# schumacherlab/ONT-TCRconsensus

Hardware: AMD Instinct MI355X
Metric: UMIs clustered/sec + banded-NW GCUPS (whole node, 1/2/4/8 MI355X) (higher is better)
Workload: dtype int16/int32

## Files before the change

ont-tcrconsensus_amd/csrc/cluster_ctx.h:

```cpp
#pragma once
#include <hip/hip_runtime.h>

#include <atomic>
#include <cstdlib>
#include <cstring>
#include <memory>
#include <thread>
#include <utility>
#include <vector>

#include "ctx.h"
#include "plan.h"
#include "resolve.h"

struct umiclust_ctx;

namespace uc {

constexpr int32_t kDelta = 8192;
constexpr int32_t kDepth = 2;
constexpr int32_t kBlockMin = 2048;
constexpr int32_t kDirectRecQ = 4096;
constexpr int32_t kSpecThr = 30;
constexpr int32_t kLazyPermille = 5;
constexpr int32_t kRbDirect = 4096;

struct DebugSums {
  struct {
    double wait = 0, hq_copy = 0, rec_copy = 0, classify = 0, inorder = 0, enqueue = 0, total = 0, appends = 0,
           round_b = 0, resolve_block = 0;
  } t;
  struct {
    double dev_s = 0, trips = 0, launches = 0, pairs = 0;
  } rb;
  int64_t mispredicted = 0, saved = 0, blocked = 0;
  int64_t q_no_record = 0, q_earlier_only = 0, q_in_block = 0, q_host_ns = 0;
  int64_t s_inline = 0, s_many_relevant = 0, s_record_read = 0, s_peers_scanned = 0;
};

struct Tile {
  DevBuf<uint32_t> hist;
  DevBuf<uint32_t> off;
  DevBuf<uint32_t> cursor;
  DevBuf<uint32_t> partial;
  uint64_t post_base = 0;
  size_t post_cap = 0;
  int32_t n = 0;
  int32_t base = 0;
  int32_t seg = 0;
  int32_t len = 0;
  int32_t built_n = -1;
  bool prebuilt = false;
};

struct Pass {
  int32_t q0 = 0, nq = 0, w0 = 0;
  bool live = false;
  bool rec_direct = false;
  PinBuf<TileView> h_tiles;
  DevBuf<TileView> d_tiles;
  DevBuf<uint32_t> d_top_seqno;
  DevBuf<uint8_t> d_top_count, d_ntop;
  DevBuf<uint32_t> d_pcand, d_units;
  DevBuf<uint8_t> d_pncand, d_ppeer_count, d_pnpeer;
  DevBuf<uint32_t> d_ppost;
  DevBuf<uint16_t> d_ppeer_id;
  DevBuf<uint16_t> d_peer_id;
  DevBuf<uint8_t> d_peer_count, d_npeer;
  bool ctr_zeroed = false;
  DevBuf<uint32_t> d_counters;
// ... 80 lines not shown
  std::vector<int32_t> bin_s;
  int32_t cur_bin = -1;

  DevBuf<char> d_ascii;
  DevBuf<int64_t> d_offs;
  DevBuf<int32_t> d_perm;
  DevBuf<uint32_t> d_codes;
  DevBuf<uint8_t> d_lens;
  DevBuf<uint16_t> d_kmers;
  DevBuf<uint8_t> d_nk;
  DevBuf<char> d_masked;
  DevBuf<int32_t> d_iota;
  size_t iota_n = 0;
  bool staged = false;
  std::vector<uint32_t> rec_len;
  PinBuf<int32_t> h_perm;
  DevBuf<uint32_t> d_amb;
  PinBuf<uint32_t> h_amb;
  int64_t n_changed = 0;
  DevBuf<uint8_t> d_mchg;
  PinBuf<uint16_t> h_xm;
  DevBuf<uint16_t> d_xm;
  std::vector<int32_t> hqbin;
  DevBuf<int32_t> d_qbin, d_bin_seq0, d_bin_ord0;
  PinBuf<int32_t> h_bin_ord0;
  bool pack_on = false;
  DevBuf<uint8_t> d_acc;
  DevBuf<uint16_t> d_rank;
  std::vector<uint8_t> h_acc;
  std::vector<uint16_t> h_rank;
  uc::Index ix{this};
  uc::Pass pass[uc::kPeerTiles];
  uc::Tile blk_tile[uc::kPeerTiles + 1], solo_tile;
  uc::Tile round_tile[2];
  uc::Event a_ev[4][2];
  hipStream_t ix_st = nullptr;
  uc::Event ix_done;
  hipEvent_t last_r_ev = nullptr;
  std::unique_ptr<uc::WorkPool> pool;
  std::thread in_release;
  void join_release() {
    if (in_release.joinable()) in_release.join();
  }
  int32_t pass_B = 0;
  uc::Stream st_b, st_copy;
  PinBuf<uint32_t> h_bpq, h_bpt, h_bres;
  uc::Stream st_al;
  int32_t last_a_slot = -1;
  uc::Event evb[2];
  DevBuf<uint32_t> d_bpq, d_bpt, d_bres;

  std::vector<int32_t> cno;
  std::vector<uint8_t> strand;
  std::vector<int32_t> target;
  std::vector<int32_t> ocl;
  int32_t nclusters = 0;
  uc::ClusterNumbers num;
  std::vector<char> cons;
  std::vector<int64_t> cons_off;
  struct BinOut {
    bool done = false;
    int32_t K = 0;
    std::vector<char> cons;
    std::vector<int64_t> cons_off;
  };
  std::vector<BinOut> bout;
  bool rec_direct = false;
// ... 39 lines not shown

namespace uc {

extern std::atomic<int> g_live_ctx;

int affinity_cpus();
int pool_threads(const umiclust_ctx* c);
hipError_t main_stream_priority(umiclust_ctx* c, int level);
void ensure_traceback_buffers(umiclust_ctx* c, int32_t n);
void launch_tracebacks(umiclust_ctx* c, const DevSeqs& ds, const Scoring& sc, const TracePlan& tp, int32_t maxl,
                       hipStream_t stq);
void ensure_consensus_inputs(umiclust_ctx* c, int32_t n, int32_t K);
constexpr const char* kConsOverMsg = "consensus: %d clusters exceed the MSA column budget";
int32_t run_consensus(umiclust_ctx* c, const DevSeqs& ds, int32_t n, int32_t K, hipEvent_t ev);
void cluster_pinned(umiclust_ctx* c, int32_t bin, bool multi_bin = false, int32_t npk = 1);

struct ClusterRun {
  umiclust_ctx* const c;
  const int32_t bin, npk;
  const bool multi_bin;
  const double t0 = now_s();
  const int32_t s0, s1, n;
  std::vector<uint8_t> state_buf;
  StateView state;
  BlockPlan plan;
  std::vector<int32_t> pending;
  std::vector<int32_t> new_cents;
  bool lazy = false;
  double t_pf = 0, t_al = 0, t_host = 0, t_cons = 0;
  int32_t tw_n = 0;
  int32_t tw_maxl = kMaxLen;
  DevSeqs ds{};
  const int32_t T4;
  const int D;

  ClusterRun(umiclust_ctx* ctx, int32_t bin_, int32_t npk_, bool multi)
      : c(ctx), bin(bin_), npk(npk_), multi_bin(multi), s0(ctx->bin_s[bin_]), s1(ctx->bin_s[bin_ + npk_]), n(s1 - s0),
        T4(ctx->o4_T), D(T4 ? 2 : kDepth) {}

  void reset_bin();
  void plan_blocks();
  void alloc_traceback();
  int32_t rstart(int32_t q) const;
  void sync_index(int32_t X);
  void round_window(int32_t q, const Tile** prevs, int& nprev, int slot);
  void keep_new_cents();
  void count_lazy(int32_t k, int32_t ahead);
  void run_alone(int32_t q0, int32_t nq);
  Tile& tile_of(int32_t k) { return c->blk_tile[k % (D + 1)]; }
  void enqueue(int32_t k, int nprev);
  void prebuild_peer(int32_t k);
  void run_whole();
  Tile& stile(int32_t j) { return c->blk_tile[j % (kPeerTiles + 1)]; }
  void build_peer(int32_t j, bool side);
  void second_half(int32_t j, int32_t first, bool after_count, PfCapture* cap = nullptr);
  void count_half(int32_t j, int32_t first, int flag);
  void prime(int32_t r);
  void run_split();
  void run_pipeline();
  void drain();
  void tw_launch(int32_t lo, int32_t hi, hipStream_t stq);
  void trace_members();
  void number();
  void consensus();
  void store_outputs();
  void report_pf_prof();
  void report_debug() const;
  void report();
};

inline size_t tile_cap(int64_t nseq) {
  const int64_t raw = nseq * kMaxKmers;
  return (size_t)((raw + 7 * std::min<int64_t>(kBins, raw) + 64) & ~int64_t(7));
}
void build_tile(umiclust_ctx* c, Tile& t, const int32_t* map, int32_t first, int32_t n, int32_t xoff, int32_t vbase,
                int32_t seg_mod, hipStream_t st = nullptr);
inline TileView view_of(const Tile& t) {
  TileView v;
  v.off = t.off.p;
  v.post_base = t.post_base;
  v.n = t.n;
  v.base = t.base;
  v.seg = t.seg;
  v.len = t.len;
// ... 47 lines not shown
```

ont-tcrconsensus_amd/csrc/driver.cpp:

```cpp
#include <algorithm>
#include <cstdio>
#include <sched.h>

#include "cluster_ctx.h"

using namespace uc;

std::atomic<int> uc::g_live_ctx{0};

int uc::affinity_cpus() {
  cpu_set_t set;
  if (sched_getaffinity(0, sizeof set, &set) != 0) return io::host_cpus();
  return std::max(1, std::min(CPU_COUNT(&set), io::host_cpus()));
}

int uc::pool_threads(const umiclust_ctx* c) {
  const int want = c->tun.resolve_threads > 0 ? c->tun.resolve_threads : (g_live_ctx.load() > 1 ? 4 : 8);
  return std::max(1, std::min(want, affinity_cpus()));
}

namespace {

struct L3Pin {
  cpu_set_t saved;
// ... 101 lines not shown
    c->hip(hipMemcpyAsync(c->h_craw.p, c->t_cons.p, (size_t)K * kConsCap, hipMemcpyDeviceToHost, c->st), "d2h");
  }
  c->hip(hipMemcpyAsync(c->h_over.p, c->t_over.p, 4, hipMemcpyDeviceToHost, c->st), "d2h");
  c->hip(hipStreamSynchronize(c->st), "sync");
  return *c->h_over.p;
}


void ClusterRun::reset_bin() {
  c->pack_on = npk > 1;
  c->cur_bin = bin;
  std::fill(c->cno.begin() + s0, c->cno.begin() + s1, -1);
  std::fill(c->strand.begin() + s0, c->strand.begin() + s1, 0);
  std::fill(c->target.begin() + s0, c->target.begin() + s1, -1);
  c->nclusters = 0;
  c->ix.reset(n);
  c->stats = umiclust_stats{};
  c->stats.n_input = c->bin_in[bin + npk] - c->bin_in[bin];
  if (c->pack_on) {
    for (int32_t b = bin; b < bin + npk; b++) c->h_bin_ord0.p[b] = INT32_MAX;
    c->hip(hipMemcpyAsync(c->d_bin_ord0.p + bin, c->h_bin_ord0.p + bin, (size_t)npk * 4, hipMemcpyHostToDevice, c->st),
           "h2d bin ord0");
  }
  c->stats.n_kept = n;
  state_buf.assign((size_t)n, ST_UNDET);
  state = StateView{state_buf.data(), s0};
  if (c->tun.walk_dump) c->wd.assign((size_t)n * 4, -1);
}

void ClusterRun::plan_blocks() {
  int32_t B = std::max(1, std::min<int32_t>(c->tun.block_size, kMaxBlock));
  if (c->tun.block_div > 0) B = std::min<int32_t>(B, std::max<int32_t>(kBlockMin, ((s1 - s0) / c->tun.block_div + 255) & ~255));
  c->pass_B = B;
  for (Pass& P : c->pass) ensure_pass_buffers(c, P, B);
  plan.hlen = c->hlen.data();
  plan.s0 = s0;
  plan.s1 = s1;
  plan.B = B;
  plan.mix = c->tun.mix_len > 0 || (c->tun.mix_len < 0 && (B < kMaxBlock || c->pack_on));
  plan.o4_T = T4;
  plan.hqbin = c->pack_on ? c->hqbin.data() : nullptr;
  plan.bin_s = c->bin_s.data();
  plan.regrow = c->tun.regrow;
  plan.start(c->b_hint);
}

void ClusterRun::alloc_traceback() {
  c->t_opsidx.assign(n, -1);
  ensure_traceback_buffers(c, n);
  ds = dev_seqs(c);
  tw_maxl = traceback_maxl(c->hlen.data(), s0, s1);
}

int32_t ClusterRun::rstart(int32_t q) const { return round_start(c, s0, q); }
void ClusterRun::sync_index(int32_t X) {
  size_t m = 0;
  while (m < pending.size() && pending[m] < X) m++;
  if (!m) return;
  std::vector<int32_t> a(pending.begin(), pending.begin() + (ptrdiff_t)m);
  c->ix.append(a);
  pending.erase(pending.begin(), pending.begin() + (ptrdiff_t)m);
}
void ClusterRun::round_window(int32_t q, const Tile** prevs, int& nprev, int slot) {
  const int32_t first = nprev ? prevs[0]->base : q;
  const int32_t W = rstart(first);
  if (W < first) {
    Tile& rt = c->round_tile[slot & 1];
    build_tile(c, rt, c->d_iota.p, W, first - W, 0, (kPeerTiles - 1) * kPeerRegion, 1 << 30);
    rt.base = W;
    rt.seg = kPeerTiles - 1;
    rt.len = 0;
    rt.prebuilt = false;
    for (int i = nprev; i > 0; i--) prevs[i] = prevs[i - 1];
    prevs[0] = &rt;
    nprev++;
  }
  sync_index(W);
}

void ClusterRun::keep_new_cents() {
  if (T4) pending.insert(pending.end(), new_cents.begin(), new_cents.end());
  else c->ix.append(new_cents);
  c->stats.n_blocks++;
}
void ClusterRun::count_lazy(int32_t k, int32_t ahead) {
  lazy = (int64_t)new_cents.size() * 1000 < (int64_t)plan.blocks[k].second * kLazyPermille;
  c->stats.n_lazy_passes += (lazy && k + ahead < plan.nb()) ? 1 : 0;
}
void ClusterRun::run_alone(int32_t q0, int32_t nq) {
  Pass& P = c->pass[0];
  int32_t piece = nq;
  for (int32_t q = q0; q < q0 + nq;) {
    const int32_t m = std::min(piece, q0 + nq - q);
    const Tile* prevs[kPeerTiles];
    int nprev = 0;
    if (T4) round_window(q, prevs, nprev, 0);
    enqueue_pass(c, P, q, m, prevs, nprev, c->solo_tile, 0);
    c->stats.n_reruns++;
    int32_t done = 0;
    const bool all = resolve_pass(c, P, state, new_cents, t_pf, t_al, t_host, &done);
    if (done > 0) {
      keep_new_cents();
      q += done;
    }
    if (!all && done == 0) {
      if (m == 1) c->fail(UMICLUST_EDEVICE, "peer overflow with block of 1");
      piece = std::max(1, m / 2);
    }
  }
}

void ClusterRun::enqueue(int32_t k, int nprev) {
  const Tile* prevs[kPeerTiles];
  for (int i = 0; i < nprev; i++) prevs[i] = &tile_of(k - nprev + i);
  if (T4) round_window(plan.blocks[k].first, prevs, nprev, k);
  enqueue_pass(c, c->pass[k % D], plan.blocks[k].first, plan.blocks[k].second, prevs, nprev, tile_of(k), k % D, lazy);
}
void ClusterRun::prebuild_peer(int32_t k) {
  const auto& blk = plan.blocks[k + D];
  Tile& t = tile_of(k + D);
  hipStream_t bst = multi_bin ? nullptr : (hipStream_t)c->st_b;
  if (bst) {
    c->hip(hipStreamWaitEvent(bst, c->pass[k % D].ev[1], 0), "wait");
    c->pt_ev.get(c, hipEventDisableTiming);
  }
  build_tile(c, t, c->d_iota.p, blk.first, blk.second, 0, ((k + D) % D) * kPeerRegion, 1 << 30, bst);
  if (bst) {
    c->hip(hipEventRecord(c->pt_ev, bst), "event");
    c->pt_pending = true;
  }
  t.base = blk.first;
  t.seg = (k + D) % D;
  t.prebuilt = true;
}
void ClusterRun::run_whole() {
  for (int32_t i = 0; i < D && i < plan.nb(); i++) enqueue(i, i);
  for (int32_t k = 0; k < plan.nb(); k++) {
    Pass& P = c->pass[k % D];
    const double te0 = now_s();
    if (k + D < plan.nb()) prebuild_peer(k);
    c->dbg.t.enqueue += now_s() - te0;
    int32_t done = 0;
    if (!resolve_pass(c, P, state, new_cents, t_pf, t_al, t_host, &done)) {
      for (int i = 1; i < D; i++) {
        Pass& Q = c->pass[(k + i) % D];
        if (Q.live) {
          c->hip(hipEventSynchronize(Q.ev[4]), "sync");
          Q.live = false;
        }
      }
      if (done > 0) keep_new_cents();
      run_alone(plan.blocks[k].first + done, plan.blocks[k].second - done);
      plan.overflowed(k);
      for (int i = 1; i <= D; i++)
        if (k + i < plan.nb()) enqueue(k + i, i - 1);
      continue;
    }
    keep_new_cents();
    count_lazy(k, D);
    if (plan.resolved(k, D, c->last_max_npeer)) {
      c->stats.n_regrows++;
      tile_of(k + D).prebuilt = false;
    }
    const double te1 = now_s();
    if (k + D < plan.nb()) enqueue(k + D, D - 1);
    c->dbg.t.enqueue += now_s() - te1;
  }
}

void ClusterRun::build_peer(int32_t j, bool side) {
  const auto& blk = plan.blocks[j];
  Tile& t = stile(j);
  const int32_t region = j % kPeerTiles;
  if (!(t.prebuilt && t.base == blk.first && t.n == blk.second && t.seg == region)) {
    hipStream_t bs = c->st;
    if (side && c->ix_st) {
      bs = c->ix_st;
      if (c->last_r_ev) c->hip(hipStreamWaitEvent(bs, c->last_r_ev, 0), "wait");
    }
    build_tile(c, t, c->d_iota.p, blk.first, blk.second, 0, region * kPeerRegion, 1 << 30, bs);
    if (bs != c->st) c->hip(hipEventRecord(c->ix_done.get(c), bs), "event");
  }
  t.base = blk.first;
  t.seg = region;
  t.len = c->hlen[blk.first];
  t.prebuilt = true;
}
void ClusterRun::second_half(int32_t j, int32_t first, bool after_count, PfCapture* cap) {
  const Tile* prevs[kPeerTiles];
  int np = 0;
  for (int32_t i = first; i < j; i++) prevs[np++] = &stile(i);
  enqueue_pass(c, c->pass[j % 2], plan.blocks[j].first, plan.blocks[j].second, prevs, np, stile(j), j % kPeerTiles, lazy,
               after_count, cap);
}
void ClusterRun::count_half(int32_t j, int32_t first, int flag) {
  const Tile* wins[kPeerTiles];
  int nw = 0;
  for (int32_t i = first; i <= j; i++) wins[nw++] = &stile(i);
// ... 114 lines not shown
  c->hip(hipMemcpy(h, c->pf_prof.p, sizeof(h), hipMemcpyDeviceToHost), "d2h");
  const double nwg = h[8] ? (double)h[8] : 1.0;
  fprintf(stderr,
          "prefilter phase clocks per workgroup (%llu): query %.0f views %.0f offsets %.0f table %.0f count %.0f "
          "scan %.0f select %.0f out %.0f\n",
          h[8], h[5] / nwg, h[6] / nwg, h[7] / nwg, h[0] / nwg, h[1] / nwg, h[2] / nwg, h[3] / nwg, h[4] / nwg);
  const double nc = h[14] ? (double)h[14] : 1.0;
  fprintf(stderr,
          "k_pf_count phase clocks per workgroup (%llu sampled): zero %.0f table %.0f count %.0f scan %.0f "
          "peers+out %.0f; chunks per workgroup %.1f; table = offsets %.0f + block scan %.0f + writes\n",
          h[14], h[9] / nc, h[10] / nc, h[11] / nc, h[12] / nc, h[13] / nc, h[15] / nc, h[16] / nc, h[17] / nc);
  if (h[19])
    fprintf(stderr, "k_pf_count sampled workgroups: %.0f shader cycles in %.2f us real time = %.2f GHz in the pipeline\n",
            h[18] / nc, h[19] / nc / 100.0, (double)h[18] / ((double)h[19] / 100e6) / 1e9);
  c->hip(hipMemset(c->pf_prof.p, 0, 24 * sizeof(unsigned long long)), "memset");
}
void ClusterRun::report_debug() const {
  const DebugSums& d = c->dbg;
  fprintf(stderr, "bin %d: n %d mispredicted %lld saved(seen) %lld blocked %lld deferred %lld\n", bin, n,
          (long long)d.mispredicted, (long long)d.saved, (long long)d.blocked, (long long)c->stats.n_deferred);
  fprintf(stderr, "bin %d: queries no-record %lld earlier-block-only %lld in-block %lld; pass-1 host %.3f s\n", bin,
          (long long)d.q_no_record, (long long)d.q_earlier_only, (long long)d.q_in_block, d.q_host_ns * 1e-9);
  fprintf(stderr, "bin %d: strands inline %lld many-relevant %lld record-read %lld peers-scanned %lld\n", bin,
          (long long)d.s_inline, (long long)d.s_many_relevant, (long long)d.s_record_read,
          (long long)d.s_peers_scanned);
  fprintf(stderr, "bin %d: resolve wait %.3f hq-copy %.3f rec-copy %.3f classify %.3f in-order %.3f total %.3f s "
          "(round B and the rest %.3f: round-B round trips %.3f, rest of resolve_block %.3f, outside it %.3f)\n", bin,
          d.t.wait, d.t.hq_copy, d.t.rec_copy, d.t.classify, d.t.inorder, d.t.total,
          d.t.total - d.t.wait - d.t.hq_copy - d.t.rec_copy - d.t.classify - d.t.inorder, d.t.round_b,
          d.t.resolve_block - d.t.classify - d.t.inorder - d.t.round_b,
          d.t.total - d.t.wait - d.t.hq_copy - d.t.rec_copy - d.t.resolve_block);
  fprintf(stderr, "bin %d: host: split-pass appends %.3f, enqueue (peer tiles, appends, launches) %.3f s; bin %.3f s\n",
          bin, d.t.appends, d.t.enqueue, now_s() - t0);
  fprintf(stderr, "bin %d: round B: %.0f round trips, %.0f launches, %.0f pairs, %.4f s between its first and last "
          "launch's events\n", bin, d.rb.trips, d.rb.launches, d.rb.pairs, d.rb.dev_s);
}
void ClusterRun::report() {
  c->stats.n_clusters = c->nclusters;
  c->stats.t_prefilter_s = t_pf;
  c->stats.t_align_s = t_al;
  c->stats.t_consensus_s = t_cons;
  c->stats.t_host_s = t_host;
  if (c->pf_prof.p) report_pf_prof();
  c->stats.t_total_s = now_s() - t0;
  c->clustered = true;
  if (c->tun.walk_dump && !c->wd.empty()) {
    if (FILE* f = fopen(c->tun.walk_dump, "wb")) {
      fwrite(c->wd.data(), 2, c->wd.size(), f);
      fclose(f);
    }
    c->wd.clear();
  }
  if (c->tun.debug) report_debug();
  c->dbg = DebugSums{};
}

static void cluster_all(umiclust_ctx* c, int32_t bin, bool multi_bin, int32_t npk) {
  c->rec_direct = g_live_ctx.load() > 1;
  if (bin < 0 || npk < 1 || bin + npk >= (int32_t)c->bin_s.size())
    c->fail(UMICLUST_EINVAL, "bins [%d, %d) out of range", bin, bin + npk);
  ClusterRun r(c, bin, npk, multi_bin);
  r.reset_bin();
  r.plan_blocks();
  c->ix.layout(r.n, r.T4);
  r.alloc_traceback();
  r.run_pipeline();
// ... 191 lines not shown
```

ont-tcrconsensus_amd/csrc/kernels.hip:

```cpp
#include <hip/hip_runtime.h>

#include <atomic>
#include <cstring>
#include <type_traits>
#include <mutex>

#include "align_kernels.h"
#include "umiclust_internal.h"

namespace uc {

enum { k_attr_prefilter = 0, k_attr_consensus = 1, k_attr_count = 2 };
constexpr int kAttrDevices = 64;
static std::atomic<bool> g_attr_set[kAttrDevices][k_attr_count];
static bool attr_set_on_device(int which) {
  int d = 0;
  if (hipGetDevice(&d) != hipSuccess || d < 0 || d >= kAttrDevices) return false;
  return g_attr_set[d][which];
}
static void mark_attr_set(int which) {
  int d = 0;
  if (hipGetDevice(&d) == hipSuccess && d >= 0 && d < kAttrDevices) g_attr_set[d][which] = true;
}

// ... 1503 lines not shown
    atomicAdd(cells, (unsigned long long)ql * tl);
    w.e = (uint8_t)b1;
  }
  if (act) ws[qs] = w;
}

hipError_t launch_walk(int32_t round, int32_t q0, int32_t nqs, int32_t both, int32_t spec_thr,
                       const uint32_t* top_seqno, const uint8_t* top_count, const uint8_t* ntop,
                       const uint8_t* lens, const uint32_t* res, const uint8_t* acc_tab,
                       const uint16_t* rank_tab, WalkState* ws, uint32_t* pq, uint32_t* pt,
                       uint32_t* outidx, const SegTab& sg, uint32_t* seg_cnt, unsigned long long* cells,
                       hipStream_t st) {
  if (nqs <= 0) return hipSuccess;
  hipLaunchKernelGGL(k_walk, dim3((nqs + 255) / 256), dim3(256), 0, st, round, q0, nqs, both, spec_thr,
                     top_seqno, top_count, ntop, lens, res, acc_tab, rank_tab, ws, pq, pt, outidx,
                     sg, seg_cnt, cells);
  return hipGetLastError();
}

__device__ __forceinline__ unsigned long long cand_key_dev(uint32_t count, uint32_t len, uint32_t seqno) {
  return ((unsigned long long)(127u - count) << 56) | ((unsigned long long)len << 48) | seqno;
}
__device__ __forceinline__ bool walk_open(const WalkState& w) {
  return (w.w % kBatch) != 0 || w.w == 0 || (!w.acc && w.w < kWalk);
}
__device__ __forceinline__ bool peer_relevant(const WalkState& w, uint32_t count, uint32_t len, uint32_t seqno) {
  return walk_open(w) || cand_key_dev(count, len, seqno) < w.lastkey;
}

__device__ __forceinline__ bool member_expected(uint32_t ps, int32_t q0, int32_t nqb, int32_t both,
                                               const WalkState* __restrict__ ws, const uint8_t* __restrict__ npeer,
                                               const WalkState* __restrict__ ws_prev,
                                               const uint8_t* __restrict__ npeer_prev, int32_t q0_prev,
                                               int32_t nq_prev) {
  (void)npeer;
  (void)npeer_prev;
  const WalkState* W;
  int32_t base;
  if ((int32_t)ps >= q0 && (int32_t)ps < q0 + nqb) {
    W = ws;
    base = q0;
  } else if (ws_prev && (int32_t)ps >= q0_prev && (int32_t)ps < q0_prev + nq_prev) {
    W = ws_prev;
    base = q0_prev;
  } else {
    return false;
  }
  for (int s = 0; s < both; s++)
    if (W[(int64_t)((int32_t)ps - base) * both + s].acc) return true;
  return false;
}

__global__ __launch_bounds__(256) void k_peer_rel(int32_t q0, int32_t w0, int32_t nqs, int32_t both,
                                                  const uint8_t* __restrict__ lens, const WalkState* __restrict__ ws,
                                                  const uint16_t* __restrict__ peer_id,
                                                  const uint8_t* __restrict__ peer_count,
                                                  const uint8_t* __restrict__ npeer,
                                                  unsigned long long* __restrict__ aligned, int32_t emit,
                                                  const WalkState* __restrict__ ws_prev,
                                                  const uint8_t* __restrict__ npeer_prev, int32_t q0_prev,
                                                  int32_t nq_prev) {
  constexpr int kPH = kPeerCap / 64;
  const int lane = threadIdx.x & 63;
  const int qs = (int)blockIdx.x * 4 + (int)(threadIdx.x >> 6);
  if (qs >= nqs) return;
  const int np = npeer[qs];
  const bool any = np != 255 && np != 0 && emit;
  const WalkState w = ws[qs];
  const int32_t nqb = nqs / both;
#pragma unroll
  for (int hh = 0; hh < kPH; hh++) {
    const int x = lane + 64 * hh;
    bool r = false;
    if (any && x < np) {
      const uint32_t ps = (uint32_t)(w0 + peer_id[(int64_t)qs * kPeerCap + x]);
      r = peer_relevant(w, peer_count[(int64_t)qs * kPeerCap + x], lens[ps], ps) &&
          !member_expected(ps, q0, nqb, both, ws, npeer, ws_prev, npeer_prev, q0_prev, nq_prev);
    }
    const unsigned long long m = __ballot(r);
    if (lane == 0) aligned[(int64_t)qs * kPH + hh] = m;
  }
}

__global__ __launch_bounds__(256) void k_peer_pairs(int32_t q0, int32_t w0, int32_t nqs, int32_t both,
                                                    const uint8_t* __restrict__ lens, const WalkState* __restrict__ ws,
                                                    const uint16_t* __restrict__ peer_id,
                                                    const uint8_t* __restrict__ peer_count, const uint8_t* __restrict__ npeer,
                                                    uint32_t* __restrict__ pq, uint32_t* __restrict__ pt,
                                                    uint32_t* __restrict__ outidx, SegTab sg, uint32_t* __restrict__ seg_cnt,
                                                    unsigned long long* __restrict__ cells, uint32_t* __restrict__ nstat,
                                                    uint32_t out0, unsigned long long* __restrict__ aligned, int32_t emit,
                                                    const WalkState* __restrict__ ws_prev,
                                                    const uint8_t* __restrict__ npeer_prev, int32_t q0_prev,
                                                    int32_t nq_prev) {
  const int qs = blockIdx.x * blockDim.x + threadIdx.x;
  const bool live = qs < nqs;
  constexpr int kPH = kPeerCap / 64;
  unsigned long long rel[kPH] = {};
  if (live)
    for (int hh = 0; hh < kPH; hh++) rel[hh] = aligned[(int64_t)qs * kPH + hh];
  const int32_t q = q0 + (live ? qs : 0) / both;
  const int ql = lens[q];
  uint32_t n = 0;
  for (int hh = 0; hh < kPH; hh++) n += (uint32_t)__builtin_popcountll(rel[hh]);
  const uint32_t si = (uint32_t)(sg.lmax - ql);
  const uint32_t k0 = seg_alloc(n, si, seg_cnt);
  if (!n) return;
  atomicAdd(nstat, n);
  uint32_t k = sg.base[si] + k0;
  const uint32_t qv = ((uint32_t)q << 1) | (uint32_t)(qs % both);
  uint32_t tl = 0;
  for (int hh = 0; hh < kPH; hh++)
    for (unsigned long long m = rel[hh]; m; m &= m - 1ull) {
      const int x = 64 * hh + __builtin_ctzll(m);
      const uint32_t t = (uint32_t)(w0 + peer_id[(int64_t)qs * kPeerCap + x]);
      pq[k] = qv;
      pt[k] = t;
      outidx[k] = out0 + (uint32_t)(qs * kPeerCap + x);
      tl += lens[t];
      k++;
    }
  atomicAdd(cells, (unsigned long long)ql * tl);
}

hipError_t launch_peer_pairs(int32_t q0, int32_t w0, int32_t nqs, int32_t both, const uint8_t* lens,
                             const WalkState* ws, const uint16_t* peer_id, const uint8_t* peer_count,
                             const uint8_t* npeer, uint32_t* pq, uint32_t* pt, uint32_t* outidx, const SegTab& sg,
                             uint32_t* seg_cnt, unsigned long long* cells, uint32_t* nstat, uint32_t out0,
                             unsigned long long* aligned, int32_t emit, const WalkState* ws_prev,
                             const uint8_t* npeer_prev, int32_t q0_prev, int32_t nq_prev, hipStream_t st) {
  if (nqs <= 0) return hipSuccess;
  hipLaunchKernelGGL(k_peer_rel, dim3((nqs + 3) / 4), dim3(256), 0, st, q0, w0, nqs, both, lens, ws, peer_id,
                     peer_count, npeer, aligned, emit, ws_prev, npeer_prev, q0_prev, nq_prev);
  hipLaunchKernelGGL(k_peer_pairs, dim3((nqs + 255) / 256), dim3(256), 0, st, q0, w0, nqs, both, lens, ws, peer_id,
                     peer_count, npeer, pq, pt, outidx, sg, seg_cnt, cells, nstat, out0, aligned, emit, ws_prev,
                     npeer_prev, q0_prev, nq_prev);
  return hipGetLastError();
}

constexpr int kPackWaves = 4, kPackQ = 4;
__global__ __launch_bounds__(64 * kPackWaves) void k_pack(int32_t nqs, int32_t w0, const uint8_t* __restrict__ lens,
                                              const WalkState* __restrict__ ws, const uint8_t* __restrict__ ntop,
                                              const uint32_t* __restrict__ top_seqno,
                                              const uint8_t* __restrict__ top_count, const uint32_t* __restrict__ res,
                                              const uint8_t* __restrict__ npeer, const uint16_t* __restrict__ peer_id,
                                              const uint8_t* __restrict__ peer_count,
                                              const uint32_t* __restrict__ peer_res,
                                              const unsigned long long* __restrict__ aligned,
                                              uint32_t* __restrict__ reccount,
                                              HostQs* __restrict__ hq, uint32_t* __restrict__ rec,
                                              uint32_t* __restrict__ counters, uint32_t* __restrict__ hcounters,
                                              uint32_t* __restrict__ hreccount) {
  __shared__ uint32_t wsize[kPackWaves * kPackQ];
  __shared__ uint32_t last_wg;
  const int lane = threadIdx.x & 63, wave = threadIdx.x >> 6;
  const int qs0 = ((int)blockIdx.x * kPackWaves + wave) * kPackQ;
  if (blockIdx.x == 0 && threadIdx.x < 64) {
    uint32_t v = threadIdx.x < kPostSpread ? counters[16 + 32 * threadIdx.x] : 0u;
#pragma unroll
    for (int d = 1; d < 64; d <<= 1) v += __shfl_xor(v, d, 64);
    if (threadIdx.x < 16) hcounters[threadIdx.x] = threadIdx.x == 0 ? v : counters[threadIdx.x];
  }
  constexpr int kH = kPeerCap / 64;
  static_assert(kPackQ * kH <= 32, "relevant / aligned bits per lane");
  uint32_t pw[kPackQ][kH], relb = 0u, alb = 0u;
#pragma unroll
  for (int i = 0; i < kPackQ; i++) {
    const int qs = qs0 + i;
    const bool live = qs < nqs;
// ... 535 lines not shown
```

ont-tcrconsensus_amd/csrc/pass.cpp:

```cpp
#include <cstdio>
#include <string>

#include "cluster_ctx.h"

namespace uc {

void ensure_pass_buffers(umiclust_ctx* c, Pass& P, int32_t B) {
  const size_t nqs = (size_t)B * c->both;
  alloc_each(c, nqs * kTopHits, P.d_top_seqno, P.d_top_count);
  c->hip(P.d_ntop.ensure(nqs), "alloc");
  c->hip(P.d_pcand.ensure(nqs * kParts * kPartCand), "alloc");
  alloc_each(c, nqs * kParts, P.d_pncand, P.d_units);
  alloc_each(c, nqs * kParts * kPeerCap, P.d_ppeer_id, P.d_ppeer_count);
  alloc_each(c, nqs * kParts, P.d_pnpeer, P.d_ppost);
  alloc_each(c, nqs * kPeerCap, P.d_peer_id, P.d_peer_count);
  c->hip(P.d_npeer.ensure(nqs), "alloc");
  c->hip(P.d_counters.ensure(kCountersLen), "alloc");
  P.ctr_zeroed = false;
  alloc_each(c, nqs * (kWalk + kPeerCap), P.d_pq, P.d_pt, P.d_outidx, P.d_res);
  c->hip(P.d_hq.ensure(nqs), "alloc");
  c->hip(P.d_paligned.ensure((size_t)nqs * (kPeerCap / 64)), "alloc");
  c->hip(P.d_ws.ensure(nqs), "alloc");
  if (!P.d_reccount.p) {
    c->hip(P.d_reccount.ensure(2), "alloc");
// ... 188 lines not shown
  const int32_t lmax = block_maxlen(c, q0, nq), nsg = lmax - block_minlen(c, q0, nq) + 1;
  if (nsg > kSegLens) c->fail(UMICLUST_EINVAL, "block spans %d query lengths (> %d)", nsg, kSegLens);
  int32_t nql[kSegLens] = {};
  for (int32_t q = q0; q < q0 + nq; q++) nql[lmax - c->hlen[q]]++;
  SegTab sg0{}, sg1{};
  sg0.lmax = sg1.lmax = lmax;
  sg0.nseg = sg1.nseg = nsg;
  for (int32_t i = 0, b0 = 0, b1 = 0; i < nsg; i++) {
    sg0.base[i] = (uint32_t)b0;
    sg1.base[i] = (uint32_t)b1;
    b0 += nql[i] * both * kWalk;
    b1 += nql[i] * both * (kWalk + kPeerCap);
  }
  uint32_t* segc = P.d_counters.p + kSegSlot;
  unsigned long long* cells_w = reinterpret_cast<unsigned long long*>(P.d_counters.p + 12);
  unsigned long long* cells_p = reinterpret_cast<unsigned long long*>(P.d_counters.p + 14);
  auto align_round = [&](const SegTab& sg, int per_qs, uint32_t* cnt, const char* what) {
    for (int32_t i = 0; i < nsg; i++)
      if (nql[i])
        c->hip(launch_align(ds, lmax - i, c->ambig, P.d_pq.p + sg.base[i], P.d_pt.p + sg.base[i], nql[i] * both * per_qs,
                            cnt + i, P.d_outidx.p + sg.base[i], c->sc, P.d_res.p, st, c->tun.band_pairs),
               what);
  };
  c->hip(launch_walk(-1, q0, nqs, both, kSpecThr, P.d_top_seqno.p, P.d_top_count.p, P.d_ntop.p, c->d_lens.p, P.d_res.p,
                     c->d_acc.p, c->d_rank.p, P.d_ws.p, P.d_pq.p, P.d_pt.p, P.d_outidx.p, sg0, segc, cells_w, st),
         "walk");
  c->hip(hipEventRecord(P.ev[2], st), "event");
  const uint32_t peer_out0 = (uint32_t)nqs * kWalk;
  align_round(sg0, kWalk, segc, "align 0");
  c->hip(launch_walk(0, q0, nqs, both, kSpecThr, P.d_top_seqno.p, P.d_top_count.p, P.d_ntop.p, c->d_lens.p,
                     P.d_res.p, c->d_acc.p, c->d_rank.p, P.d_ws.p, P.d_pq.p, P.d_pt.p, P.d_outidx.p, sg1, segc + kSegLens,
                     cells_w, st),
         "walk 0");
  const Pass* prev = nullptr;
  for (const Pass& Q : c->pass)
    if (&Q != &P && Q.nq > 0 && Q.q0 + Q.nq == q0) prev = &Q;
  c->hip(launch_peer_pairs(q0, w0, nqs, both, c->d_lens.p, P.d_ws.p, P.d_peer_id.p, P.d_peer_count.p, P.d_npeer.p,
                           P.d_pq.p, P.d_pt.p, P.d_outidx.p, sg1, segc + kSegLens, cells_p, P.d_counters.p + 8,
                           peer_out0, P.d_paligned.p, lazy_peers ? 0 : 1,
                           prev ? prev->d_ws.p : nullptr, prev ? prev->d_npeer.p : nullptr, prev ? prev->q0 : 0,
                           prev ? prev->nq : 0, st),
         "peer pairs");
  align_round(sg1, kWalk + kPeerCap, segc + kSegLens, "align 1");
  c->hip(launch_walk(1, q0, nqs, both, kSpecThr, P.d_top_seqno.p, P.d_top_count.p, P.d_ntop.p, c->d_lens.p,
                     P.d_res.p, c->d_acc.p, c->d_rank.p, P.d_ws.p, P.d_pq.p, P.d_pt.p, P.d_outidx.p, sg1,
                     segc + 2 * kSegLens, cells_w, st),
         "walk 1");
  c->hip(hipEventRecord(P.ev[3], st), "event");
  P.rec_direct = c->rec_direct || nq <= kDirectRecQ;
  c->hip(launch_pack(nqs, w0, c->d_lens.p, P.d_ws.p, P.d_ntop.p, P.d_top_seqno.p, P.d_top_count.p, P.d_res.p,
                     P.d_npeer.p, P.d_peer_id.p, P.d_peer_count.p, P.d_res.p + peer_out0, P.d_paligned.p, P.d_reccount.p,
                     P.rec_direct ? P.h_hq.p : P.d_hq.p,
                     P.rec_direct ? P.h_rec.p : P.d_rec.p, P.d_counters.p, P.h_counters.p, P.h_reccount.p, st),
         "pack");
  P.ctr_zeroed = nqs > 0;
  if (!P.rec_direct) {
    c->hip(hipMemcpyAsync(P.h_hq.p, P.d_hq.p, (size_t)nqs * sizeof(HostQs), hipMemcpyDeviceToHost, st), "d2h outcomes");
    const size_t est = std::min<size_t>(P.rec_est, P.d_rec.n);
    c->hip(hipMemcpyAsync(P.h_rec.p, P.d_rec.p, est * 4, hipMemcpyDeviceToHost, st), "d2h records");
  }
  c->hip(hipEventRecord(P.ev[4], st), "event");
}

void enqueue_count(umiclust_ctx* c, Pass& P, int32_t q0, int32_t nq, const Tile* const* wins, int nwin, int flag,
                   int32_t slot) {
  P.a_live = false;
  if (c->ix.nseg() > 1) return;
  hipStream_t st = c->st;
  wait_index_and_tiles(c, st);
  if (c->ix_st) c->hip(hipStreamWaitEvent(st, P.ev[1], 0), "wait");
  c->hip(hipEventSynchronize(P.ev_a), "sync");
  const int32_t nv = c->ix.stage_views(P.h_tiles_a, P.d_tiles_a, st);
  c->hip(hipEventRecord(P.ev_a, st), "event");
  PrefilterArgs a = prefilter_args(c, P, P.h_tiles_a.p, P.d_tiles_a.p, nv, q0, nq);
// ... 262 lines not shown
```

ont-tcrconsensus_amd/csrc/umiclust_internal.h:

```cpp
#pragma once
#include <hip/hip_runtime.h>
#include <stdint.h>

#include "umiclust_consts.h"

namespace uc {

struct Scoring {
  int32_t match, mismatch;
  int32_t go[6], ge[6];
  int32_t boundary_open;
};

struct TileView {
  const uint32_t* off;
  uint64_t post_base;
  int32_t n;
  int32_t base;
  int32_t seg;
  int32_t len;
};

struct DevSeqs {
  const uint32_t* codes;
// ... 78 lines not shown
bool prefilter_one_wave(const PrefilterArgs& a);

hipError_t launch_align(const DevSeqs& s, int32_t qlen, bool ambig, const uint32_t* pq, const uint32_t* pt, int32_t npairs,
                        const uint32_t* dev_npairs, const uint32_t* outidx, const Scoring& sc,
                        uint32_t* out, hipStream_t st, int32_t band_max = 0);

struct WalkState {
  unsigned long long lastkey;
  uint32_t best_t;
  uint32_t cells;
  uint16_t best_rank;
  uint8_t w;
  uint8_t done;
  uint8_t acc;
  uint8_t e;
  uint8_t pad[2];
};
struct SegTab {
  int32_t lmax;
  int32_t nseg;
  uint32_t base[kSegLens];
};
hipError_t launch_walk(int32_t round, int32_t q0, int32_t nqs, int32_t both, int32_t spec_thr,
                       const uint32_t* top_seqno, const uint8_t* top_count, const uint8_t* ntop,
                       const uint8_t* lens, const uint32_t* res, const uint8_t* acc_tab,
                       const uint16_t* rank_tab, WalkState* ws, uint32_t* pq, uint32_t* pt,
                       uint32_t* outidx, const SegTab& sg, uint32_t* seg_cnt, unsigned long long* cells,
                       hipStream_t st);
hipError_t launch_peer_pairs(int32_t q0, int32_t w0, int32_t nqs, int32_t both, const uint8_t* lens,
                             const WalkState* ws, const uint16_t* peer_id, const uint8_t* peer_count,
                             const uint8_t* npeer, uint32_t* pq, uint32_t* pt, uint32_t* outidx, const SegTab& sg,
                             uint32_t* seg_cnt, unsigned long long* cells, uint32_t* nstat, uint32_t out0,
                             unsigned long long* aligned, int32_t emit, const WalkState* ws_prev,
                             const uint8_t* npeer_prev, int32_t q0_prev, int32_t nq_prev, hipStream_t st);
hipError_t launch_pack(int32_t nqs, int32_t w0, const uint8_t* lens, const WalkState* ws, const uint8_t* ntop,
                       const uint32_t* top_seqno, const uint8_t* top_count, const uint32_t* res,
                       const uint8_t* npeer, const uint16_t* peer_id, const uint8_t* peer_count,
                       const uint32_t* peer_res, const unsigned long long* aligned, uint32_t* reccount, HostQs* hq,
                       uint32_t* rec, uint32_t* counters, uint32_t* hcounters, uint32_t* hreccount, hipStream_t st);
hipError_t launch_traceback(const DevSeqs& s, const uint32_t* pq, const uint32_t* pt, int32_t npairs,
                            const Scoring& sc, uint8_t* ops, uint16_t* nops, uint32_t* out, hipStream_t st,
                            int32_t maxl, int32_t maxq = 0);
hipError_t launch_consensus(const DevSeqs& s, const int32_t* cstart, int32_t nclusters,
                            const int32_t* member_seqno, const int32_t* member_opsidx,
                            const uint8_t* member_strand, const uint8_t* ops,
                            const uint16_t* nops, char* cons, uint16_t* conslen,
                            int32_t* overflow, hipStream_t st);

struct OvBuffers {
  uint64_t* hash;
  int32_t* region;
  unsigned long long* keys;
  unsigned long long* rep;
  int64_t* slot;
  uint32_t* cnt;
  uint32_t* start;
  uint32_t* cursor;
  uint32_t* bsum;
  uint32_t* members;
  uint32_t* collision;
  uint32_t* big;
  uint32_t* nbig;
};
constexpr int kOvSmallBucket = 32;
hipError_t launch_overlap_table(const char* seqs, const int64_t* offs, int64_t n, const int64_t* rstart, int32_t nreg,
                                uint64_t seed, uint64_t hmask, uint64_t mask, const OvBuffers& B, bool csr,
                                uint32_t* collided, hipStream_t st);
// ... 142 lines not shown
```

Before: 5.293 million.

## Deepen the whole-bin pass pipeline to three in-flight blocks in o4 mode

When o4 rounding is on, the bin is single and blocks are smaller than the max, the whole-bin pipeline keeps three passes in flight instead of two. Enqueueing moves into enqueue_due, which postpones a pass when a round tile would not fit. Round tiles now take a free peer region, and the peer-pair kernels can see the walk state of a second earlier pass. The aim is to hide more host resolve latency behind device work, at the cost of more tile-region bookkeeping, a fallback to depth two on overflow, and extra branches in the peer kernels.

```diff
diff --git a/ont-tcrconsensus_amd/csrc/cluster_ctx.h b/ont-tcrconsensus_amd/csrc/cluster_ctx.h
--- a/ont-tcrconsensus_amd/csrc/cluster_ctx.h
+++ b/ont-tcrconsensus_amd/csrc/cluster_ctx.h
@@ -19,6 +19,8 @@
 
 constexpr int32_t kDelta = 8192;
 constexpr int32_t kDepth = 2;
+constexpr int32_t kDepthO4 = 3;
+static_assert(kDepthO4 <= 3, "a window holds at most kPeerTiles blocks");
 constexpr int32_t kBlockMin = 2048;
 constexpr int32_t kDirectRecQ = 4096;
 constexpr int32_t kSpecThr = 30;
@@ -36,6 +38,7 @@
   int64_t mispredicted = 0, saved = 0, blocked = 0;
   int64_t q_no_record = 0, q_earlier_only = 0, q_in_block = 0, q_host_ns = 0;
   int64_t s_inline = 0, s_many_relevant = 0, s_record_read = 0, s_peers_scanned = 0;
+  int64_t n_postponed = 0, n_round_tiles = 0, n_depth_drops = 0;
 };
 
 struct Tile {
@@ -182,7 +185,7 @@
   uc::Index ix{this};
   uc::Pass pass[uc::kPeerTiles];
   uc::Tile blk_tile[uc::kPeerTiles + 1], solo_tile;
-  uc::Tile round_tile[2];
+  uc::Tile round_tile[uc::kPeerTiles];
   uc::Event a_ev[4][2];
   hipStream_t ix_st = nullptr;
   uc::Event ix_done;
@@ -288,24 +291,27 @@
   int32_t tw_maxl = kMaxLen;
   DevSeqs ds{};
   const int32_t T4;
-  const int D;
+  int D;
+  int32_t next_enq = 0;
 
   ClusterRun(umiclust_ctx* ctx, int32_t bin_, int32_t npk_, bool multi)
       : c(ctx), bin(bin_), npk(npk_), multi_bin(multi), s0(ctx->bin_s[bin_]), s1(ctx->bin_s[bin_ + npk_]), n(s1 - s0),
-        T4(ctx->o4_T), D(T4 ? 2 : kDepth) {}
+        T4(ctx->o4_T), D(kDepth) {}
 
   void reset_bin();
   void plan_blocks();
   void alloc_traceback();
   int32_t rstart(int32_t q) const;
   void sync_index(int32_t X);
-  void round_window(int32_t q, const Tile** prevs, int& nprev, int slot);
+  bool mid_round(int32_t q) const { return rstart(q) < q; }
+  void round_window(int32_t q, const Tile** prevs, int& nprev, int slot, unsigned used);
   void keep_new_cents();
   void count_lazy(int32_t k, int32_t ahead);
   void run_alone(int32_t q0, int32_t nq);
   Tile& tile_of(int32_t k) { return c->blk_tile[k % (D + 1)]; }
   void enqueue(int32_t k, int nprev);
   void prebuild_peer(int32_t k);
+  void enqueue_due(int32_t k, bool steady);
   void run_whole();
   Tile& stile(int32_t j) { return c->blk_tile[j % (kPeerTiles + 1)]; }
   void build_peer(int32_t j, bool side);
diff --git a/ont-tcrconsensus_amd/csrc/driver.cpp b/ont-tcrconsensus_amd/csrc/driver.cpp
--- a/ont-tcrconsensus_amd/csrc/driver.cpp
+++ b/ont-tcrconsensus_amd/csrc/driver.cpp
@@ -157,6 +157,7 @@
   int32_t B = std::max(1, std::min<int32_t>(c->tun.block_size, kMaxBlock));
   if (c->tun.block_div > 0) B = std::min<int32_t>(B, std::max<int32_t>(kBlockMin, ((s1 - s0) / c->tun.block_div + 255) & ~255));
   c->pass_B = B;
+  D = (T4 && !multi_bin && B < kMaxBlock) ? kDepthO4 : kDepth;
   for (Pass& P : c->pass) ensure_pass_buffers(c, P, B);
   plan.hlen = c->hlen.data();
   plan.s0 = s0;
@@ -186,14 +187,18 @@
   c->ix.append(a);
   pending.erase(pending.begin(), pending.begin() + (ptrdiff_t)m);
 }
-void ClusterRun::round_window(int32_t q, const Tile** prevs, int& nprev, int slot) {
+void ClusterRun::round_window(int32_t q, const Tile** prevs, int& nprev, int slot, unsigned used) {
   const int32_t first = nprev ? prevs[0]->base : q;
   const int32_t W = rstart(first);
   if (W < first) {
-    Tile& rt = c->round_tile[slot & 1];
-    build_tile(c, rt, c->d_iota.p, W, first - W, 0, (kPeerTiles - 1) * kPeerRegion, 1 << 30);
+    int region = kPeerTiles - 1;
+    while (region >= 0 && (used >> region & 1u)) region--;
+    if (region < 0 || nprev + 2 > kPeerTiles) c->fail(UMICLUST_EDEVICE, "internal: no room for the round tile");
+    Tile& rt = c->round_tile[slot % kPeerTiles];
+    build_tile(c, rt, c->d_iota.p, W, first - W, 0, region * kPeerRegion, 1 << 30);
+    c->dbg.n_round_tiles++;
     rt.base = W;
-    rt.seg = kPeerTiles - 1;
+    rt.seg = region;
     rt.len = 0;
     rt.prebuilt = false;
     for (int i = nprev; i > 0; i--) prevs[i] = prevs[i - 1];
@@ -210,7 +215,7 @@
 }
 void ClusterRun::count_lazy(int32_t k, int32_t ahead) {
   lazy = (int64_t)new_cents.size() * 1000 < (int64_t)plan.blocks[k].second * kLazyPermille;
-  c->stats.n_lazy_passes += (lazy && k + ahead < plan.nb()) ? 1 : 0;
+  c->stats.n_lazy_passes += (lazy && ahead > 0 && k + ahead < plan.nb()) ? 1 : 0;
 }
 void ClusterRun::run_alone(int32_t q0, int32_t nq) {
   Pass& P = c->pass[0];
@@ -219,7 +224,7 @@
     const int32_t m = std::min(piece, q0 + nq - q);
     const Tile* prevs[kPeerTiles];
     int nprev = 0;
-    if (T4) round_window(q, prevs, nprev, 0);
+    if (T4) round_window(q, prevs, nprev, 0, 1u);
     enqueue_pass(c, P, q, m, prevs, nprev, c->solo_tile, 0);
     c->stats.n_reruns++;
     int32_t done = 0;
@@ -237,16 +242,30 @@
 
 void ClusterRun::enqueue(int32_t k, int nprev) {
   const Tile* prevs[kPeerTiles];
+  unsigned used = 0;
+  for (int i = 0; i <= nprev; i++) used |= 1u << ((k - i) % D);
   for (int i = 0; i < nprev; i++) prevs[i] = &tile_of(k - nprev + i);
-  if (T4) round_window(plan.blocks[k].first, prevs, nprev, k);
+  if (T4) round_window(plan.blocks[k].first, prevs, nprev, k, used);
   enqueue_pass(c, c->pass[k % D], plan.blocks[k].first, plan.blocks[k].second, prevs, nprev, tile_of(k), k % D, lazy);
+}
+void ClusterRun::enqueue_due(int32_t k, bool steady) {
+  const int32_t oldest = k + 1;
+  for (; next_enq < plan.nb() && next_enq <= k + D; next_enq++) {
+    const int nprev = next_enq - oldest;
+    if (T4 && nprev + 2 > kPeerTiles && mid_round(plan.blocks[oldest].first)) {
+      c->dbg.n_postponed++;
+      break;
+    }
+    enqueue(next_enq, nprev);
+    c->stats.n_lazy_passes += (steady && lazy) ? 1 : 0;
+  }
 }
 void ClusterRun::prebuild_peer(int32_t k) {
   const auto& blk = plan.blocks[k + D];
   Tile& t = tile_of(k + D);
   hipStream_t bst = multi_bin ? nullptr : (hipStream_t)c->st_b;
   if (bst) {
-    c->hip(hipStreamWaitEvent(bst, c->pass[k % D].ev[1], 0), "wait");
+    c->hip(hipStreamWaitEvent(bst, c->pass[(k + D - 2) % D].ev[1], 0), "wait");
     c->pt_ev.get(c, hipEventDisableTiming);
   }
   build_tile(c, t, c->d_iota.p, blk.first, blk.second, 0, ((k + D) % D) * kPeerRegion, 1 << 30, bst);
@@ -259,7 +278,8 @@
   t.prebuilt = true;
 }
 void ClusterRun::run_whole() {
-  for (int32_t i = 0; i < D && i < plan.nb(); i++) enqueue(i, i);
+  next_enq = 0;
+  enqueue_due(-1, false);
   for (int32_t k = 0; k < plan.nb(); k++) {
     Pass& P = c->pass[k % D];
     const double te0 = now_s();
@@ -267,8 +287,8 @@
     c->dbg.t.enqueue += now_s() - te0;
     int32_t done = 0;
     if (!resolve_pass(c, P, state, new_cents, t_pf, t_al, t_host, &done)) {
-      for (int i = 1; i < D; i++) {
-        Pass& Q = c->pass[(k + i) % D];
+      for (int32_t j = k + 1; j < next_enq; j++) {
+        Pass& Q = c->pass[j % D];
         if (Q.live) {
           c->hip(hipEventSynchronize(Q.ev[4]), "sync");
           Q.live = false;
@@ -277,18 +297,22 @@
       if (done > 0) keep_new_cents();
       run_alone(plan.blocks[k].first + done, plan.blocks[k].second - done);
       plan.overflowed(k);
-      for (int i = 1; i <= D; i++)
-        if (k + i < plan.nb()) enqueue(k + i, i - 1);
+      if (D > kDepth) {
+        D = kDepth;
+        c->dbg.n_depth_drops++;
+      }
+      next_enq = k + 1;
+      enqueue_due(k, false);
       continue;
     }
     keep_new_cents();
-    count_lazy(k, D);
+    count_lazy(k, 0);
     if (plan.resolved(k, D, c->last_max_npeer)) {
       c->stats.n_regrows++;
       tile_of(k + D).prebuilt = false;
     }
     const double te1 = now_s();
-    if (k + D < plan.nb()) enqueue(k + D, D - 1);
+    enqueue_due(k, true);
     c->dbg.t.enqueue += now_s() - te1;
   }
 }
@@ -469,6 +493,8 @@
           d.t.total - d.t.wait - d.t.hq_copy - d.t.rec_copy - d.t.resolve_block);
   fprintf(stderr, "bin %d: host: split-pass appends %.3f, enqueue (peer tiles, appends, launches) %.3f s; bin %.3f s\n",
           bin, d.t.appends, d.t.enqueue, now_s() - t0);
+  fprintf(stderr, "bin %d: whole passes: depth %d at the end, depth-drops %lld, postponed passes %lld, round tiles %lld\n",
+          bin, D, (long long)d.n_depth_drops, (long long)d.n_postponed, (long long)d.n_round_tiles);
   fprintf(stderr, "bin %d: round B: %.0f round trips, %.0f launches, %.0f pairs, %.4f s between its first and last "
           "launch's events\n", bin, d.rb.trips, d.rb.launches, d.rb.pairs, d.rb.dev_s);
 }
diff --git a/ont-tcrconsensus_amd/csrc/kernels.hip b/ont-tcrconsensus_amd/csrc/kernels.hip
--- a/ont-tcrconsensus_amd/csrc/kernels.hip
+++ b/ont-tcrconsensus_amd/csrc/kernels.hip
@@ -1559,7 +1559,8 @@
                                                const WalkState* __restrict__ ws, const uint8_t* __restrict__ npeer,
                                                const WalkState* __restrict__ ws_prev,
                                                const uint8_t* __restrict__ npeer_prev, int32_t q0_prev,
-                                               int32_t nq_prev) {
+                                               int32_t nq_prev, const WalkState* __restrict__ ws_prev2,
+                                               int32_t q0_prev2, int32_t nq_prev2) {
   (void)npeer;
   (void)npeer_prev;
   const WalkState* W;
@@ -1570,6 +1571,9 @@
   } else if (ws_prev && (int32_t)ps >= q0_prev && (int32_t)ps < q0_prev + nq_prev) {
     W = ws_prev;
     base = q0_prev;
+  } else if (ws_prev2 && (int32_t)ps >= q0_prev2 && (int32_t)ps < q0_prev2 + nq_prev2) {
+    W = ws_prev2;
+    base = q0_prev2;
   } else {
     return false;
   }
@@ -1586,7 +1590,8 @@
                                                   unsigned long long* __restrict__ aligned, int32_t emit,
                                                   const WalkState* __restrict__ ws_prev,
                                                   const uint8_t* __restrict__ npeer_prev, int32_t q0_prev,
-                                                  int32_t nq_prev) {
+                                                  int32_t nq_prev, const WalkState* __restrict__ ws_prev2,
+                                                  int32_t q0_prev2, int32_t nq_prev2) {
   constexpr int kPH = kPeerCap / 64;
   const int lane = threadIdx.x & 63;
   const int qs = (int)blockIdx.x * 4 + (int)(threadIdx.x >> 6);
@@ -1602,7 +1607,8 @@
     if (any && x < np) {
       const uint32_t ps = (uint32_t)(w0 + peer_id[(int64_t)qs * kPeerCap + x]);
       r = peer_relevant(w, peer_count[(int64_t)qs * kPeerCap + x], lens[ps], ps) &&
-          !member_expected(ps, q0, nqb, both, ws, npeer, ws_prev, npeer_prev, q0_prev, nq_prev);
+          !member_expected(ps, q0, nqb, both, ws, npeer, ws_prev, npeer_prev, q0_prev, nq_prev, ws_prev2,
+                          q0_prev2, nq_prev2);
     }
     const unsigned long long m = __ballot(r);
     if (lane == 0) aligned[(int64_t)qs * kPH + hh] = m;
@@ -1619,7 +1625,8 @@
                                                     uint32_t out0, unsigned long long* __restrict__ aligned, int32_t emit,
                                                     const WalkState* __restrict__ ws_prev,
                                                     const uint8_t* __restrict__ npeer_prev, int32_t q0_prev,
-                                                    int32_t nq_prev) {
+                                                    int32_t nq_prev, const WalkState* __restrict__ ws_prev2,
+                                                    int32_t q0_prev2, int32_t nq_prev2) {
   const int qs = blockIdx.x * blockDim.x + threadIdx.x;
   const bool live = qs < nqs;
   constexpr int kPH = kPeerCap / 64;
@@ -1655,13 +1662,15 @@
                              const uint8_t* npeer, uint32_t* pq, uint32_t* pt, uint32_t* outidx, const SegTab& sg,
                              uint32_t* seg_cnt, unsigned long long* cells, uint32_t* nstat, uint32_t out0,
                              unsigned long long* aligned, int32_t emit, const WalkState* ws_prev,
-                             const uint8_t* npeer_prev, int32_t q0_prev, int32_t nq_prev, hipStream_t st) {
+                             const uint8_t* npeer_prev, int32_t q0_prev, int32_t nq_prev, const WalkState* ws_prev2,
+                             int32_t q0_prev2, int32_t nq_prev2, hipStream_t st) {
   if (nqs <= 0) return hipSuccess;
   hipLaunchKernelGGL(k_peer_rel, dim3((nqs + 3) / 4), dim3(256), 0, st, q0, w0, nqs, both, lens, ws, peer_id,
-                     peer_count, npeer, aligned, emit, ws_prev, npeer_prev, q0_prev, nq_prev);
+                     peer_count, npeer, aligned, emit, ws_prev, npeer_prev, q0_prev, nq_prev, ws_prev2, q0_prev2,
+                     nq_prev2);
   hipLaunchKernelGGL(k_peer_pairs, dim3((nqs + 255) / 256), dim3(256), 0, st, q0, w0, nqs, both, lens, ws, peer_id,
                      peer_count, npeer, pq, pt, outidx, sg, seg_cnt, cells, nstat, out0, aligned, emit, ws_prev,
-                     npeer_prev, q0_prev, nq_prev);
+                     npeer_prev, q0_prev, nq_prev, ws_prev2, q0_prev2, nq_prev2);
   return hipGetLastError();
 }
 
diff --git a/ont-tcrconsensus_amd/csrc/pass.cpp b/ont-tcrconsensus_amd/csrc/pass.cpp
--- a/ont-tcrconsensus_amd/csrc/pass.cpp
+++ b/ont-tcrconsensus_amd/csrc/pass.cpp
@@ -244,14 +244,18 @@
                      P.d_res.p, c->d_acc.p, c->d_rank.p, P.d_ws.p, P.d_pq.p, P.d_pt.p, P.d_outidx.p, sg1, segc + kSegLens,
                      cells_w, st),
          "walk 0");
-  const Pass* prev = nullptr;
+  const Pass *prev = nullptr, *prev2 = nullptr;
   for (const Pass& Q : c->pass)
     if (&Q != &P && Q.nq > 0 && Q.q0 + Q.nq == q0) prev = &Q;
+  if (prev)
+    for (const Pass& Q : c->pass)
+      if (&Q != &P && &Q != prev && Q.nq > 0 && Q.q0 + Q.nq == prev->q0) prev2 = &Q;
   c->hip(launch_peer_pairs(q0, w0, nqs, both, c->d_lens.p, P.d_ws.p, P.d_peer_id.p, P.d_peer_count.p, P.d_npeer.p,
                            P.d_pq.p, P.d_pt.p, P.d_outidx.p, sg1, segc + kSegLens, cells_p, P.d_counters.p + 8,
                            peer_out0, P.d_paligned.p, lazy_peers ? 0 : 1,
                            prev ? prev->d_ws.p : nullptr, prev ? prev->d_npeer.p : nullptr, prev ? prev->q0 : 0,
-                           prev ? prev->nq : 0, st),
+                           prev ? prev->nq : 0, prev2 ? prev2->d_ws.p : nullptr, prev2 ? prev2->q0 : 0,
+                           prev2 ? prev2->nq : 0, st),
          "peer pairs");
   align_round(sg1, kWalk + kPeerCap, segc + kSegLens, "align 1");
   c->hip(launch_walk(1, q0, nqs, both, kSpecThr, P.d_top_seqno.p, P.d_top_count.p, P.d_ntop.p, c->d_lens.p,
diff --git a/ont-tcrconsensus_amd/csrc/umiclust_internal.h b/ont-tcrconsensus_amd/csrc/umiclust_internal.h
--- a/ont-tcrconsensus_amd/csrc/umiclust_internal.h
+++ b/ont-tcrconsensus_amd/csrc/umiclust_internal.h
@@ -134,7 +134,8 @@
                              const uint8_t* npeer, uint32_t* pq, uint32_t* pt, uint32_t* outidx, const SegTab& sg,
                              uint32_t* seg_cnt, unsigned long long* cells, uint32_t* nstat, uint32_t out0,
                              unsigned long long* aligned, int32_t emit, const WalkState* ws_prev,
-                             const uint8_t* npeer_prev, int32_t q0_prev, int32_t nq_prev, hipStream_t st);
+                             const uint8_t* npeer_prev, int32_t q0_prev, int32_t nq_prev, const WalkState* ws_prev2,
+                             int32_t q0_prev2, int32_t nq_prev2, hipStream_t st);
 hipError_t launch_pack(int32_t nqs, int32_t w0, const uint8_t* lens, const WalkState* ws, const uint8_t* ntop,
                        const uint32_t* top_seqno, const uint8_t* top_count, const uint32_t* res,
                        const uint8_t* npeer, const uint16_t* peer_id, const uint8_t* peer_count,
```

Result: slower. 5.230 million (-1.2%).
